# Aidenryan/GF_ORB_SLAM

Hardware: AMD Instinct MI355X
Metric: front-end fps (extract+match+GF-select) @ 752x480/1000 feats; pose-opt ms/iter (higher is better)
Workload: dtype u8/int32 (extract, match), f64 (GF, pose LM)

## Files before the change

### gf_orb_slam_amd/csrc/extract.hip

```cpp
#include <math.h>
#include <string.h>

#include <algorithm>
#include <cfloat>
#include <cmath>
#include <vector>

#include "common.h"
#include "libm_sincosf.h"
#include "orb_pattern.h"
#include "select.h"

#define GF_MAX_LEVELS 12

namespace {

__constant__ uint32_t c_pattern8[256];
__constant__ uint32_t c_ic_tab[256];

struct LevelGeom {
    int nlevels;
    int w[GF_MAX_LEVELS], h[GF_MAX_LEVELS];
    int pw[GF_MAX_LEVELS];
    long long off[GF_MAX_LEVELS];
// ... 601 lines not shown
            q[2] = row3(i2 * pitch + rsh[i2]);
        }
        int ie = rowi(ya + 2), se = rsh[ie];
        auto step = [&](int y, R3& u, R3& c, R3& d, R3& e) {
            e = row3(ie * pitch + se);
            const int in = rowi(y + 3);
            se = rsh[in];
            ie = in;
            const int mx = max(max(max(u.a, u.b), max(u.c, c.a)), max(max(c.c, d.a), max(d.b, d.c)));
            const bool keep = okc && c.b != 0 && c.b > mx;
            if (keep) atomicOr(&bits[(y * dw + x) >> 5], 1u << ((y * dw + x) & 31));
            cnt += __popcll(__ballot(keep));
        };
        for (int y = ya; y < yb; y += 4) {
            step(y, q[0], q[1], q[2], q[3]);
            if (y + 1 < yb) step(y + 1, q[1], q[2], q[3], q[0]);
            if (y + 2 < yb) step(y + 2, q[2], q[3], q[0], q[1]);
            if (y + 3 < yb) step(y + 3, q[3], q[0], q[1], q[2]);
        }
    }
    return cnt;
}

#ifndef FC_THREADS
#define FC_THREADS 256
#endif
constexpr int FC_NT = FC_THREADS, FC_NW = FC_THREADS / 64;
static_assert(FC_NT == 64 || FC_NT == 256 || FC_NT == 512, "k_fast_cells: 1, 4 or 8 waves");

template <int NW>
__device__ int block_scan_nw(int v, int* tmp, int& total) {
    const int lane = threadIdx.x & 63, wid = threadIdx.x >> 6;
    int wt;
    const int x = wave_scan_excl(v, wt);
    if (lane == 0) tmp[wid] = wt;
    __syncthreads();
    int base = 0;
    total = 0;
#pragma unroll
    for (int i = 0; i < NW; i++) {
        base += i < wid ? tmp[i] : 0;
        total += tmp[i];
    }
    __syncthreads();
    return base + x;
}
__device__ __forceinline__ void fc_sync() {
    if constexpr (FC_NT == 64) {
        __builtin_amdgcn_fence(__ATOMIC_RELEASE, "wavefront");
        __builtin_amdgcn_wave_barrier();
        __builtin_amdgcn_fence(__ATOMIC_ACQUIRE, "wavefront");
    } else {
        __syncthreads();
    }
}

struct FcLayout {
    int nq, ndw, pitch, wpr, nwords;
    size_t sc_bytes, bits_bytes, total;
};
__host__ __device__ inline FcLayout fc_layout(int dw, int dh, int w, int h) {
    FcLayout L;
    L.nq = (dw + 3) / 4;
    L.ndw = L.nq + 2;
    L.pitch = 4 * L.ndw;
    L.wpr = (dw + 31) / 32;
    L.nwords = dh * L.wpr;
    L.sc_bytes = (size_t)(dh + 2) * L.pitch;
    L.bits_bytes = 4 * (size_t)((L.nwords + 3) & ~3);
    L.total = L.sc_bytes + L.bits_bytes + (size_t)w * h;
    return L;
}

template <int NWV>
__device__ __forceinline__ int cell_nms4(const uint32_t* sc32, const FcLayout& Ly, uint32_t* bits, int dh, int th) {
    typedef unsigned short u2 __attribute__((ext_vector_type(2)));
    const int lane = threadIdx.x & 63, wv = threadIdx.x >> 6;
// ... 26 lines not shown
            const u2 vE = __builtin_elementwise_max(u.e, d.e), vO = __builtin_elementwise_max(u.o, d.o);
            const u2 vEL = __builtin_elementwise_max(u.el, d.el), vOR = __builtin_elementwise_max(u.orr, d.orr);
            const u2 mxE = __builtin_elementwise_max(__builtin_elementwise_max(vE, vEL),
                                                     __builtin_elementwise_max(vO, __builtin_elementwise_max(c.el, c.o)));
            const u2 mxO = __builtin_elementwise_max(__builtin_elementwise_max(vO, vOR),
                                                     __builtin_elementwise_max(vE, __builtin_elementwise_max(c.e, c.orr)));
            const u2 kE = __builtin_elementwise_min(__builtin_elementwise_sub_sat(c.e, mxE), ONE);
            const u2 kO = __builtin_elementwise_min(__builtin_elementwise_sub_sat(c.o, mxO), ONE);
            const uint32_t t = __builtin_bit_cast(uint32_t, kE) | (__builtin_bit_cast(uint32_t, kO) << 1);
            const uint32_t m = okq ? ((t & 3u) | ((t >> 14) & 12u)) : 0u;
            if (m) atomicOr(brow + (y - ya) * Ly.wpr, m << sh);
            cnt += __popc(m);
        };
        Q q0 = rowq(ya), q1 = rowq(ya + 1), q2;
        for (int y = ya; y < yb; y += 3) {
            step(y, q0, q1, q2);
            if (y + 1 < yb) step(y + 1, q1, q2, q0);
            if (y + 2 < yb) step(y + 2, q2, q0, q1);
        }
    }
    return gfd::warp_sum(cnt);
}

template <typename E>
__global__ __launch_bounds__(FC_NT) void k_fast_cells(Planes P, LevelGeom g, const uint8_t* __restrict__ score,
                                                    const CellInfo* __restrict__ cells, E* __restrict__ lists,
                                                    long long list_stride, int* __restrict__ counts, int fast_th,
                                                    int min_th) {
    gfd::ext_prio();
    extern __shared__ __align__(16) uint8_t smem[];
    __shared__ int s_cnt[2][FC_NW];
    __shared__ int scan_tmp[FC_NW];
    int cid, f;
    gfd::xcd_block(cid, f);
    const int tid = threadIdx.x;
    const CellInfo ci = cells[cid];
    if (ci.band) return;
    const int dw = ci.w - 6, dh = ci.h - 6;
    if (!ci.valid || dw <= 0 || dh <= 0) {
        if (tid == 0) counts[(long long)f * g.ncells + cid] = 0;
        return;
    }
    const FcLayout Ly = fc_layout(dw, dh, ci.w, ci.h);
    uint8_t* sc = smem;
    uint32_t* sc32 = reinterpret_cast<uint32_t*>(smem);
    uint32_t* bits = reinterpret_cast<uint32_t*>(smem + Ly.sc_bytes);
    const int l = ci.level, lw = g.pw[l];
    const uint8_t* SC = score + (long long)f * g.bslab + g.boff[l] + (long long)(ci.y0 + 3) * lw + ci.x0 + 3;
    {
        const uint32_t sh = (uint32_t)((uintptr_t)SC & 3u);
        const uint32_t* SCa = reinterpret_cast<const uint32_t*>((uintptr_t)SC & ~(uintptr_t)3);
        const int lw4 = lw >> 2, nrows = dh + 2;
        const int ndw = Ly.ndw, rstep = max(FC_NT / ndw, 1);
        const int j = tid % ndw, r0 = tid / ndw;
        const bool jdata = j >= 1 && j <= Ly.nq;
        uint32_t bmask = ~0u;
        if (jdata && dw - 4 * (j - 1) < 4) bmask = (1u << (8 * (dw - 4 * (j - 1)))) - 1u;
        constexpr int FC_LB = 8;
        for (int rb = r0; rb < nrows; rb += FC_LB * rstep) {
            uint32_t lo[FC_LB], hi[FC_LB];
            const int jc = min(max(j, 1), Ly.nq) - 1;
#pragma unroll
            for (int k = 0; k < FC_LB; k++) {
                const int rc = min(max(rb + k * rstep, 1), dh) - 1;
                const uint32_t* src = SCa + (long long)rc * lw4 + jc;
                lo[k] = gfd::ldg(src);
                hi[k] = gfd::ldg(src + 1);
            }
#pragma unroll
            for (int k = 0; k < FC_LB; k++) {
                const int r = rb + k * rstep;
                const bool data = jdata && r >= 1 && r <= dh;
                if (r < nrows && r0 < rstep)
                    sc32[r * ndw + j] = data ? __builtin_amdgcn_alignbyte(hi[k], lo[k], sh) & bmask : 0u;
            }
        }
    }
    for (int i = tid; i < Ly.nwords; i += FC_NT) bits[i] = 0;
    fc_sync();
    int c = cell_nms4<FC_NW>(sc32, Ly, bits, dh, fast_th);
    if ((tid & 63) == 0) s_cnt[0][tid >> 6] = c;
    fc_sync();
    int total = 0;
#pragma unroll
    for (int k = 0; k < FC_NW; k++) total += s_cnt[0][k];
    if (total <= 3) {
        uint8_t* roi = smem + Ly.sc_bytes + Ly.bits_bytes;
        int sstride;
        const uint8_t* Sl = level_plane(P, g, f, l, sstride) + (long long)ci.y0 * sstride + ci.x0;
        for (int i = tid; i < ci.w * ci.h; i += FC_NT) {
            const int r = pyr_div(i, 1.0f / (float)ci.w);
            roi[i] = gfd::ldg(Sl + (long long)r * sstride + (i - r * ci.w));
        }
        fc_sync();
        for (int i = tid; i < dw * dh; i += FC_NT) {
            const int y = pyr_div(i, 1.0f / (float)dw), x = i - y * dw;
            int cv[16];
            circle_vals(roi, ci.w, x + 3, y + 3, cv);
            const int M = fast_max_arc(roi[(y + 3) * ci.w + x + 3], cv);
            sc[(y + 1) * Ly.pitch + 4 + x] = M > min_th ? (uint8_t)M : 0;
        }
        for (int i = tid; i < Ly.nwords; i += FC_NT) bits[i] = 0;
        fc_sync();
        c = cell_nms4<FC_NW>(sc32, Ly, bits, dh, min_th);
        if ((tid & 63) == 0) s_cnt[1][tid >> 6] = c;
        fc_sync();
        total = 0;
#pragma unroll
        for (int k = 0; k < FC_NW; k++) total += s_cnt[1][k];
    }
    E* out = lists + (long long)f * list_stride + ci.cap_off;
    const int X0 = ci.x0 + 3, Y0 = ci.y0 + 3;
    int base = 0;
    for (int w0 = 0; w0 < Ly.nwords; w0 += FC_NT) {
        const int i = w0 + tid;
        uint32_t word = i < Ly.nwords ? bits[i] : 0u;
        int tot;
        int off;
        if constexpr (FC_NT == 64) {
            off = base + wave_scan_excl(__popc(word), tot);
        } else {
            off = base + block_scan_nw<FC_NW>(__popc(word), scan_tmp, tot);
        }
        if (word) {
            const int y = i / Ly.wpr, xw = 32 * (i - y * Ly.wpr);
            const uint8_t* srow = sc + (y + 1) * Ly.pitch + 4;
            while (word) {
                const int x = xw + __ffs(word) - 1;
                word &= word - 1;
                out[off++] = cell_entry<E>(srow[x] - 1, X0 + x, Y0 + y, P, g, f, l);
            }
        }
        base += tot;
    }
    if (tid == 0) counts[(long long)f * g.ncells + cid] = total;
}

template <typename E>
__global__ __launch_bounds__(256) void k_fast_cells_band(Planes P, LevelGeom g, const uint8_t* __restrict__ score,
                                                         const CellInfo* __restrict__ cells,
                                                         const int* __restrict__ band_ids, E* __restrict__ lists,
                                                         long long list_stride, int* __restrict__ counts, int fast_th,
                                                         int min_th) {
    gfd::ext_prio();
    extern __shared__ __align__(16) uint8_t smem[];
    __shared__ int s_cnt[4];
    __shared__ int scan_tmp[4];
    const int cid = band_ids[blockIdx.x], f = blockIdx.y, tid = threadIdx.x;
    const CellInfo ci = cells[cid];
    const int dw = ci.w - 6, dh = ci.h - 6, BH = ci.band;
    const int n = dw * dh, nwords = (n + 31) >> 5;
    const int ndw = (dw + 6) >> 2, pitch = 4 * ndw;
    uint32_t* bits = reinterpret_cast<uint32_t*>(smem);
    uint8_t* sc = smem + 16 * ((nwords + 3) / 4);
    uint8_t* rsh = sc + (BH + 3) * pitch;
    uint8_t* roi = rsh + ((BH + 3 + 15) & ~15);
    const int l = ci.level, lw = g.pw[l];
    const uint8_t* SC = score + (long long)f * g.bslab + g.boff[l] + (long long)(ci.y0 + 3) * lw + ci.x0 + 3;
// ... 74 lines not shown
#define SEL_MAX_CELLS 1024
#ifndef SEL_THREADS
#define SEL_THREADS 512
#endif
#define SEL_BUF 1024
#ifndef SEL_BUF_CELL
#define SEL_BUF_CELL 512
#endif
template <typename E>
struct SelWave {
    E* a;
    uint16_t *lp, *rp;
    int cap;
};
template <typename E>
constexpr size_t sel_wave_bytes(int cap) { return (size_t)cap * (sizeof(E) + 2 * sizeof(uint16_t)); }
template <typename E>
constexpr size_t sel_wave_lds() {
    return sel_wave_bytes<E>(SEL_BUF) + (SEL_THREADS / 64 - 1) * sel_wave_bytes<E>(SEL_BUF_CELL);
}
template <typename E>
constexpr size_t sel_lds(int maxnc) { return sel_wave_lds<E>() + sizeof(int) * (3 * (size_t)maxnc + 1) + (size_t)maxnc; }

__device__ __forceinline__ void wave_sync() {
    __builtin_amdgcn_fence(__ATOMIC_RELEASE, "wavefront");
    __builtin_amdgcn_wave_barrier();
    __builtin_amdgcn_fence(__ATOMIC_ACQUIRE, "wavefront");
}

template <typename E>
__device__ __forceinline__ int sel_resp(E e) { return Ent<E>::key(e); }

template <typename E>
__device__ __forceinline__ int wave_partition(const SelWave<E>& W, int lo, int hi, int P) {
    const int lane = threadIdx.x & 63;
    const unsigned long long lt = (1ull << lane) - 1ull;
    int nL = 0, nR = 0;
    for (int i0 = 0; i0 < hi - lo; i0 += 64) {
        const int i = lo + i0 + lane, j = hi - 1 - i0 - lane;
        const bool sl = i < hi && !(sel_resp(W.a[i]) > P);
        const bool sr = j >= lo && !(P > sel_resp(W.a[j]));
        const unsigned long long bl = __ballot(sl), br = __ballot(sr);
        if (sl) W.lp[nL + __popcll(bl & lt)] = (uint16_t)i;
        if (sr) W.rp[nR + __popcll(br & lt)] = (uint16_t)j;
        nL += __popcll(bl);
        nR += __popcll(br);
    }
    wave_sync();
    const int m = min(nL, nR);
    int ks = 0;
    for (int k0 = 0; k0 < m; k0 += 64) {
        const int k = k0 + lane;
// ... 411 lines not shown
        kp.angle = angle;
        kp.response = Ent<E>::response(e);
        kp.octave = l;
        kp.class_id = -1;
        kps[(long long)f * cap + k] = kp;
    }
}

}

struct gf_extractor {
    gf_ctx* ctx = nullptr;
    hipEvent_t stage_ev = nullptr;
    int stage_after = -1;
    int nfeatures = 0, nlevels = 0, fast_th = 20, min_th = 7, width = 0, height = 0, max_batch = 0;
    bool harris = false;
    float scale_factor = 1.2f;
    LevelGeom g{};
    std::vector<CellInfo> cells;
    std::vector<int> feat_per_level;
    int capacity = 0;
    long long list_stride = 0, lvl_stride = 0;
    size_t fast_lds = 0;
    size_t band_lds = 0;
    std::vector<int> band_cells;
    int* d_band = nullptr;
    int max_tiles = 0;
    uint8_t *d_pyr = nullptr, *d_blur = nullptr, *d_score = nullptr;
    uint32_t *d_xtab = nullptr, *d_ytab = nullptr;
    PyrGeom pg{};
    size_t pyr_lds = 0;
    int sel_maxnc = 0;
    int pyr_g = PYR_G;
    CellInfo* d_cells = nullptr;
    void *d_lists = nullptr, *d_lvl = nullptr;
    int *d_counts = nullptr, *d_lvl_counts = nullptr;
    uint8_t* d_img = nullptr;
    gf_keypoint* d_kps = nullptr;
    uint8_t* d_desc = nullptr;
    int* d_nout = nullptr;
    Planes last{};
};

static int cv_round_f(float v) { return (int)std::lrintf(v); }
static int cv_floor_f(float v) {
    int i = (int)v;
// ... 35 lines not shown
                 "level size out of supported range");
        if (l > 0) {
            g.off[l] = off;
            off += ((long long)g.pw[l] * g.h[l] + 255) & ~255LL;
        }
        g.boff[l] = boff;
        boff += ((long long)g.pw[l] * g.h[l] + 255) & ~255LL;
    }
    g.slab = off;
    g.bslab = boff;
    int t = 0;
    for (int l = 0; l < nl; l++) {
        g.tile_begin[l] = t;
        g.tiles_x[l] = (g.w[l] + BT_W - 1) / BT_W;
        t += g.tiles_x[l] * ((g.h[l] + BT_H - 1) / BT_H);
    }
    g.tile_begin[nl] = t;
    ex->max_tiles = t;

    ex->cells.clear();
    ex->sel_maxnc = 0;
    ex->band_cells.clear();
    ex->band_lds = 0;
    long long cap_off = 0, lvl_off = 0;
    size_t max_lds = 0;
    const float imageRatio = (float)g.w[0] / g.h[0];
    for (int l = 0; l < nl; l++) {
        const int nDesired = ex->feat_per_level[l];
        const int levelCols = (int)std::sqrt((float)nDesired / (5 * imageRatio));
        const int levelRows = (int)(imageRatio * levelCols);
        GF_CHECK(levelCols > 0 && levelRows > 0, GF_ERR_UNSUPPORTED, "level with an empty cell grid");
        const int minB = 16, maxBX = g.w[l] - 16, maxBY = g.h[l] - 16;
        const int W = maxBX - minB, H = maxBY - minB;
        const int cellW = (int)std::ceil((float)W / levelCols);
        const int cellH = (int)std::ceil((float)H / levelRows);
        const int nCells = levelRows * levelCols;
        GF_CHECK(nCells <= SEL_MAX_CELLS, GF_ERR_UNSUPPORTED, "too many cells per level");
        ex->sel_maxnc = std::max(ex->sel_maxnc, nCells);
        g.nfcell[l] = (int)std::ceil((float)nDesired / nCells);
        g.ndesired[l] = nDesired;
        g.cell_begin[l] = (int)ex->cells.size();
        g.lvl_off[l] = lvl_off;
        std::vector<int> iniXCol(levelCols, 0);
        float hY = cellH + 6;
        long long lvl_cap = 0;
        for (int i = 0; i < levelRows; i++) {
            const float iniY = minB + i * cellH - 3;
            bool rowSkip = false;
            if (i == levelRows - 1) {
                hY = maxBY + 3 - iniY;
                if (hY <= 0) rowSkip = true;
            }
            float hX = cellW + 6;
            for (int j = 0; j < levelCols; j++) {
                float iniX;
                if (i == 0) {
                    iniX = minB + j * cellW - 3;
                    iniXCol[j] = (int)iniX;
                } else
                    iniX = iniXCol[j];
                CellInfo ci{};
                ci.level = l;
                ci.valid = 0;
                if (!rowSkip) {
                    bool skip = false;
                    if (j == levelCols - 1) {
                        hX = maxBX + 3 - iniX;
                        if (hX <= 0) skip = true;
                    }
                    if (!skip) {
                        ci.x0 = (int)iniX;
                        ci.y0 = (int)iniY;
                        ci.w = (int)hX;
                        ci.h = (int)hY;
                        ci.valid = 1;
                        int dw = std::max(ci.w - 6, 0), dh = std::max(ci.h - 6, 0);
                        ci.cap = ((dw + 1) / 2) * ((dh + 1) / 2);
                        ci.cap_off = cap_off;
                        cap_off += ci.cap;
                        lvl_cap += ci.cap;
                        const size_t pitch = 4 * (size_t)((dw + 6) / 4), bits = 16 * (((size_t)dw * dh + 127) / 128);
                        const FcLayout fl = fc_layout(dw, dh, ci.w, ci.h);
                        const size_t lds = fl.total;
                        if (lds <= FC_LDS_MAX && fl.ndw <= FC_NT) {
                            max_lds = std::max(max_lds, lds);
                        } else {
                            auto band_lds = [&](size_t bh) {
                                return bits + (bh + 3) * pitch + ((bh + 3 + 15) & ~(size_t)15) + (bh + 8) * ci.w;
                            };
                            size_t bh = std::min<size_t>(dh, 64);
                            while (bh > 4 && band_lds(bh) > FC_BAND_LDS) bh /= 2;
                            GF_CHECK(band_lds(bh) <= FC_BAND_LDS, GF_ERR_UNSUPPORTED,
                                     "cell window too large even for the banded FAST kernel");
                            ci.band = (int)bh;
                            ex->band_cells.push_back((int)ex->cells.size());
                            ex->band_lds = std::max(ex->band_lds, band_lds(bh));
                        }
                        GF_CHECK(ci.x0 >= 0 && ci.y0 >= 0 && ci.x0 + ci.w <= g.w[l] && ci.y0 + ci.h <= g.h[l],
                                 GF_ERR_ARG, "cell ROI outside level");
                    }
                }
                ex->cells.push_back(ci);
            }
        }
        lvl_off += std::max(lvl_cap, (long long)nDesired);
    }
    g.cell_begin[nl] = (int)ex->cells.size();
    g.lvl_off[nl] = lvl_off;
    g.ncells = (int)ex->cells.size();
    ex->list_stride = cap_off;
    ex->lvl_stride = lvl_off;
    ex->fast_lds = max_lds;
    ex->capacity = 0;
    for (int l = 0; l < nl; l++) ex->capacity += ex->feat_per_level[l];
    return GF_OK;
}

static void resize_tables(int sw, int sh, int dw, int dh, std::vector<int2>& xt, std::vector<int2>& yt) {
    const int ONE = 2048;
    double scale_x = 1. / ((double)dw / sw), scale_y = 1. / ((double)dh / sh);
    xt.resize(dw);
    yt.resize(dh);
    for (int dx = 0; dx < dw; dx++) {
        float fx = (float)((dx + 0.5) * scale_x - 0.5);
        int sx = cv_floor_f(fx);
        fx -= sx;
        if (sx < 0) fx = 0, sx = 0;
        if (sx >= sw - 1) fx = 0, sx = sw - 1;
        int a0 = (short)cv_round_f((1.f - fx) * ONE), a1 = (short)cv_round_f(fx * ONE);
        xt[dx] = make_int2(sx, (a0 & 0xffff) | (a1 << 16));
    }
    for (int dy = 0; dy < dh; dy++) {
        float fy = (float)((dy + 0.5) * scale_y - 0.5);
        int sy = cv_floor_f(fy);
        fy -= sy;
        int b0 = (short)cv_round_f((1.f - fy) * ONE), b1 = (short)cv_round_f(fy * ONE);
        yt[dy] = make_int2(sy, (b0 & 0xffff) | (b1 << 16));
// ... 55 lines not shown
                    const PyrSpan& a = spx[(size_t)l * nbx + kx];
                    const PyrSpan& b = spy[(size_t)l * nby + ky];
                    const size_t pitch = (size_t)((a.hi - a.lo + 1 + 8 + 3) & ~3);
                    buf[l & 1] = std::max(buf[l & 1], pitch * (size_t)(b.hi - b.lo + 1));
                }
        buf[0] = (buf[0] + 15) & ~(size_t)15;
        if (mx <= 256 && buf[0] + buf[1] <= 64 * 1024) {
            pg.nbx = nbx;
            pg.nby = nby;
            pg.lds_a = (int)buf[0];
            lds = buf[0] + buf[1];
            return true;
        }
        if (mx > 256 || (double)g.w[0] / nbx >= (double)g.h[0] / nby) nbx++;
        else nby++;
    }
    return false;
}

static void free_extractor(gf_extractor* ex) {
    (void)hipFree(ex->d_pyr);
    (void)hipFree(ex->d_blur);
    (void)hipFree(ex->d_score);
    (void)hipFree(ex->d_xtab);
    (void)hipFree(ex->d_ytab);
    (void)hipFree(ex->d_cells);
    (void)hipFree(ex->d_band);
    (void)hipFree(ex->d_lists);
    (void)hipFree(ex->d_lvl);
    (void)hipFree(ex->d_counts);
    (void)hipFree(ex->d_lvl_counts);
    (void)hipFree(ex->d_img);
    (void)hipFree(ex->d_kps);
    (void)hipFree(ex->d_desc);
    (void)hipFree(ex->d_nout);
}

static int upload_constants(int device) {
    static unsigned long long done_mask = 0;
    if (done_mask & (1ull << device)) return GF_OK;
    {
        uint32_t p8[256];
        for (int i = 0; i < 256; i++) {
            uint32_t v = 0;
            for (int j = 0; j < 4; j++) {
                const int c = kOrbPattern31[4 * i + j];
// ... 45 lines not shown
    GF_CHECK(score_type == 0 || score_type == 1, GF_ERR_ARG, "scoreType: 0 HARRIS_SCORE, 1 FAST_SCORE");
    GF_CHECK(nlevels >= 1 && nlevels <= GF_MAX_LEVELS, GF_ERR_ARG, "nlevels out of range");
    GF_CHECK(nfeatures > 0 && scale_factor > 1.f && width > 0 && height > 0 && max_batch > 0, GF_ERR_ARG,
             "bad extractor parameters");
    GF_CHECK(fast_th >= 0 && fast_th < 255, GF_ERR_ARG, "bad FAST threshold");
    GF_HIP(hipSetDevice(ctx->device));
    int rc = upload_constants(ctx->device);
    if (rc) return rc;
    gf_extractor* ex = new gf_extractor();
    ex->ctx = ctx;
    ex->nfeatures = nfeatures;
    ex->scale_factor = scale_factor;
    ex->nlevels = nlevels;
    ex->fast_th = fast_th;
    ex->width = width;
    ex->height = height;
    ex->max_batch = max_batch;
    ex->harris = score_type == 0;
    rc = plan_extractor(ex);
    if (rc) {
        delete ex;
        return rc;
    }
    const LevelGeom& g = ex->g;
    auto cleanup = [&](hipError_t e) {
        free_extractor(ex);
        delete ex;
        return gf::fail(GF_ERR_HIP, std::string("extractor alloc: ") + hipGetErrorString(e));
    };
    hipError_t e;
#define ALLOC(p, bytes)                              \
    if ((e = hipMalloc((void**)&(p), (bytes))) != hipSuccess) return cleanup(e);
    ALLOC(ex->d_pyr, std::max<long long>(g.slab, 256) * max_batch);
    ALLOC(ex->d_blur, g.bslab * max_batch);
    ALLOC(ex->d_score, g.bslab * max_batch);
    ALLOC(ex->d_cells, sizeof(CellInfo) * ex->cells.size());
    const size_t esz = ex->harris ? sizeof(uint64_t) : sizeof(uint32_t);
    ALLOC(ex->d_lists, esz * ex->list_stride * max_batch);
    ALLOC(ex->d_lvl, esz * ex->lvl_stride * max_batch);
    ALLOC(ex->d_band, sizeof(int) * std::max<size_t>(ex->band_cells.size(), 1));
    ALLOC(ex->d_counts, sizeof(int) * g.ncells * max_batch);
    ALLOC(ex->d_lvl_counts, sizeof(int) * nlevels * max_batch);
    ALLOC(ex->d_img, (size_t)width * height);
    ALLOC(ex->d_kps, sizeof(gf_keypoint) * ex->capacity);
    ALLOC(ex->d_desc, 32 * (size_t)ex->capacity);
    ALLOC(ex->d_nout, sizeof(int));
    std::vector<std::vector<int2>> xts(nlevels), yts(nlevels);
    for (int l = 1; l < nlevels; l++) resize_tables(g.w[l - 1], g.h[l - 1], g.w[l], g.h[l], xts[l], yts[l]);
    std::vector<PyrSpan> spx, spy;
    if (nlevels > 1 && !pyr_plan(g, xts, yts, ex->pg, spx, spy, ex->pyr_lds)) {
        free_extractor(ex);
        delete ex;
        return gf::fail(GF_ERR_UNSUPPORTED, "scale factor too large for the pyramid blocks");
    }
    for (int l = 1; l < nlevels && ex->pyr_g > 1; l++)
        for (int k = 0; k < ex->pg.nbx; k++) {
            const PyrSpan& sp = spx[(size_t)l * ex->pg.nbx + k];
            for (int x0 = sp.lo; x0 <= sp.hi; x0 += PYR_G)
// ... 67 lines not shown
        }
        if (!ok) {
            free_extractor(ex);
            delete ex;
            return gf::fail(GF_ERR_UNSUPPORTED, "pyramid tables outside the k_pyramid record ranges");
        }
        ex->pg.rx = pack(rx, xrec);
        ex->pg.ry = pack(ry, yrec);
        ex->pg.lds_img = (int)((ex->pyr_lds + 15) & ~(size_t)15);
        ex->pyr_lds = ex->pg.lds_img + sizeof(uint32_t) * (size_t)(ex->pg.rx + ex->pg.ry);
    }
    ALLOC(ex->d_xtab, sizeof(uint32_t) * std::max<size_t>(xrec.size(), 1));
    ALLOC(ex->d_ytab, sizeof(uint32_t) * std::max<size_t>(yrec.size(), 1));
#undef ALLOC
    if (!xrec.empty()) {
        GF_HIP(hipMemcpy(ex->d_xtab, xrec.data(), sizeof(uint32_t) * xrec.size(), hipMemcpyHostToDevice));
        GF_HIP(hipMemcpy(ex->d_ytab, yrec.data(), sizeof(uint32_t) * yrec.size(), hipMemcpyHostToDevice));
        GF_HIP(hipFuncSetAttribute((const void*)k_pyramid<PYR_G>, hipFuncAttributeMaxDynamicSharedMemorySize,
                                   (int)ex->pyr_lds));
        GF_HIP(hipFuncSetAttribute((const void*)k_pyramid<1>, hipFuncAttributeMaxDynamicSharedMemorySize,
                                   (int)ex->pyr_lds));
    }
    GF_HIP(hipMemcpy(ex->d_cells, ex->cells.data(), sizeof(CellInfo) * ex->cells.size(), hipMemcpyHostToDevice));
    if (!ex->band_cells.empty())
        GF_HIP(hipMemcpy(ex->d_band, ex->band_cells.data(), sizeof(int) * ex->band_cells.size(),
                         hipMemcpyHostToDevice));
    if (ex->harris) {
        GF_HIP(hipFuncSetAttribute((const void*)k_select_cells<uint64_t>, hipFuncAttributeMaxDynamicSharedMemorySize,
                                   (int)(SEL_CW * sel_cell_wave_lds<uint64_t>(ex->sel_maxnc))));
        GF_HIP(hipFuncSetAttribute((const void*)k_fast_cells<uint64_t>, hipFuncAttributeMaxDynamicSharedMemorySize,
                                   (int)ex->fast_lds));
        GF_HIP(hipFuncSetAttribute((const void*)k_fast_cells_band<uint64_t>,
                                   hipFuncAttributeMaxDynamicSharedMemorySize, (int)ex->band_lds));
    } else {
        GF_HIP(hipFuncSetAttribute((const void*)k_select_cells<uint32_t>, hipFuncAttributeMaxDynamicSharedMemorySize,
                                   (int)(SEL_CW * sel_cell_wave_lds<uint32_t>(ex->sel_maxnc))));
        GF_HIP(hipFuncSetAttribute((const void*)k_fast_cells<uint32_t>, hipFuncAttributeMaxDynamicSharedMemorySize,
                                   (int)ex->fast_lds));
        GF_HIP(hipFuncSetAttribute((const void*)k_fast_cells_band<uint32_t>,
                                   hipFuncAttributeMaxDynamicSharedMemorySize, (int)ex->band_lds));
    }
    *out = ex;
    return GF_OK;
}

int gf_extractor_destroy(gf_extractor* ex) {
    if (!ex) return GF_OK;
    (void)hipSetDevice(ex->ctx->device);
    free_extractor(ex);
    delete ex;
    return GF_OK;
}

int gf_extractor_info(gf_extractor* ex, int* nlevels, float* scale_factor, int* features_per_level) {
    GF_CHECK(ex, GF_ERR_ARG, "null extractor");
    if (nlevels) *nlevels = ex->nlevels;
    if (scale_factor) *scale_factor = ex->scale_factor;
    if (features_per_level)
        for (int l = 0; l < ex->nlevels; l++) features_per_level[l] = ex->feat_per_level[l];
    return GF_OK;
// ... 44 lines not shown
                GF_LAUNCH(k_pyramid<1>, dim3(ex->pg.nbx * ex->pg.nby, nframes), PYR_NT, ex->pyr_lds, s, P, g, ex->pg,
                          ex->d_xtab, ex->d_ytab);
        }
    }
    if (ex->stage_ev && ex->stage_after == 0) GF_HIP(hipEventRecord(ex->stage_ev, s));
    {
        GF_PROF(ctx, s, "k_blur_fast");
        GF_LAUNCH(k_blur_fast, dim3(ex->max_tiles, nframes), 256, 0, s, P, g, ex->d_score, ex->fast_th);
    }
    if (ex->stage_ev && ex->stage_after == 1) GF_HIP(hipEventRecord(ex->stage_ev, s));
    return ex->harris ? select_describe<uint64_t>(ex, nframes, P, d_kps, d_desc, d_counts, cap, s)
                      : select_describe<uint32_t>(ex, nframes, P, d_kps, d_desc, d_counts, cap, s);
}

template <typename E>
static int select_describe(gf_extractor* ex, int nframes, Planes P, gf_keypoint* d_kps, uint8_t* d_desc,
                           int32_t* d_counts, int cap, hipStream_t s) {
    const LevelGeom& g = ex->g;
    gf_ctx* ctx = ex->ctx;
    E* lists = reinterpret_cast<E*>(ex->d_lists);
    E* lvl = reinterpret_cast<E*>(ex->d_lvl);
    {
        GF_PROF(ctx, s, "k_fast_cells");
        GF_LAUNCH(k_fast_cells<E>, dim3(g.ncells, nframes), FC_NT, ex->fast_lds, s, P, g, ex->d_score, ex->d_cells,
                  lists, ex->list_stride, ex->d_counts, ex->fast_th, ex->min_th);
        if (!ex->band_cells.empty())
            GF_LAUNCH(k_fast_cells_band<E>, dim3((int)ex->band_cells.size(), nframes), 256, ex->band_lds, s, P, g,
                      ex->d_score, ex->d_cells, ex->d_band, lists, ex->list_stride, ex->d_counts, ex->fast_th,
                      ex->min_th);
    }
    if (ex->stage_ev && ex->stage_after == 2) GF_HIP(hipEventRecord(ex->stage_ev, s));
    {
        GF_PROF(ctx, s, "k_select");
        GF_LAUNCH(k_select_cells<E>, dim3((g.ncells + SEL_CW - 1) / SEL_CW, nframes), 64 * SEL_CW,
                  SEL_CW * sel_cell_wave_lds<E>(ex->sel_maxnc), s, g, ex->d_cells, lists, ex->list_stride,
                  ex->d_counts, lvl, ex->lvl_stride, ex->d_lvl_counts, ex->sel_maxnc);
        GF_LAUNCH(k_select_level<E>, dim3(nframes, ex->nlevels), 64, sel_wave_bytes<E>(SEL_BUF), s, g, lvl,
                  ex->lvl_stride, ex->d_lvl_counts);
    }
    if (ex->stage_ev && ex->stage_after == 3) GF_HIP(hipEventRecord(ex->stage_ev, s));
    {
        GF_PROF(ctx, s, "k_describe");
        GF_LAUNCH(k_describe<E>, dim3((ex->capacity + 7) / 8, nframes), 256, 0, s, P, g, lvl, ex->lvl_stride,
                  ex->d_lvl_counts, d_kps, d_desc, d_counts, cap);
    }
    if (ex->stage_ev && ex->stage_after == 4) GF_HIP(hipEventRecord(ex->stage_ev, s));
    GF_HIP(hipGetLastError());
    return GF_OK;
// ... 79 lines not shown
```

Baseline: 127,100.

## Split FAST cell NMS into global tiled NMS, wave-per-cell listing, and retry kernel

Replaces the block-per-cell k_fast_cells kernel with three stages. A tiled k_nms_tiles kernel computes 3x3 NMS survivors over whole level rows into a global bitmask using DPP neighbour exchange and buffer loads. A wave-per-cell k_cell_lists kernel then compacts those survivors into per-cell lists. Cells with too few corners are queued to a separate k_cell_retry kernel that reruns FAST at the lower threshold. This removes per-cell LDS staging and block-wide syncs from the common path, at the cost of extra launches, a survivor bitmap in global memory, and host-side planning that requires non-overlapping cell windows.

After: 132,000, median of 6. 3.8% higher.

```diff
diff --git a/gf_orb_slam_amd/csrc/extract.hip b/gf_orb_slam_amd/csrc/extract.hip
--- a/gf_orb_slam_amd/csrc/extract.hip
+++ b/gf_orb_slam_amd/csrc/extract.hip
@@ -647,12 +647,6 @@
     return cnt;
 }
 
-#ifndef FC_THREADS
-#define FC_THREADS 256
-#endif
-constexpr int FC_NT = FC_THREADS, FC_NW = FC_THREADS / 64;
-static_assert(FC_NT == 64 || FC_NT == 256 || FC_NT == 512, "k_fast_cells: 1, 4 or 8 waves");
-
 template <int NW>
 __device__ int block_scan_nw(int v, int* tmp, int& total) {
     const int lane = threadIdx.x & 63, wid = threadIdx.x >> 6;
@@ -670,14 +664,10 @@
     __syncthreads();
     return base + x;
 }
-__device__ __forceinline__ void fc_sync() {
-    if constexpr (FC_NT == 64) {
-        __builtin_amdgcn_fence(__ATOMIC_RELEASE, "wavefront");
-        __builtin_amdgcn_wave_barrier();
-        __builtin_amdgcn_fence(__ATOMIC_ACQUIRE, "wavefront");
-    } else {
-        __syncthreads();
-    }
+__device__ __forceinline__ void wave_sync() {
+    __builtin_amdgcn_fence(__ATOMIC_RELEASE, "wavefront");
+    __builtin_amdgcn_wave_barrier();
+    __builtin_amdgcn_fence(__ATOMIC_ACQUIRE, "wavefront");
 }
 
 struct FcLayout {
@@ -750,118 +740,302 @@
     return gfd::warp_sum(cnt);
 }
 
+#define NMS_ROWS 32
+#define NMS_PF 4
+struct NmsTask {
+    int level, q0, y0, nrows;
+    uint32_t in, up, dn;
+    int xoff;
+};
+
+__global__ __launch_bounds__(256) void k_nms_tiles(LevelGeom g, const uint8_t* __restrict__ score,
+                                                   const NmsTask* __restrict__ tasks, int ntasks,
+                                                   const uint32_t* __restrict__ xtab, uint32_t* __restrict__ surv,
+                                                   int th, int* __restrict__ retry) {
+    gfd::ext_prio();
+    typedef unsigned short u2 __attribute__((ext_vector_type(2)));
+    if (blockIdx.x == 0 && blockIdx.y == 0 && threadIdx.x == 0) retry[0] = 0;
+    int blk, f;
+    gfd::xcd_block(blk, f);
+    const int lane = threadIdx.x & 63;
+    const int t = __builtin_amdgcn_readfirstlane(4 * blk + (int)(threadIdx.x >> 6));
+    if (t >= ntasks) return;
+    const NmsTask tk = tasks[t];
+    const int l = tk.level, pw = g.pw[l], nq = pw >> 2, h = g.h[l];
+    const int q = tk.q0 + lane;
+    const bool okq = q < nq;
+    const int qc = min(q, nq - 1);
+    const int qh = lane == 0 ? q - 1 : q + 1;
+    const int qhc = ((lane == 0 || lane == 63) && qh >= 0 && qh < nq) ? qh : qc;
+    const uint32_t xm = okq ? gfd::ldg(xtab + tk.xoff + qc) : 0u;
+    auto pair16 = [](uint32_t b, int i, int j) {
+        return ((b >> i) & 1u ? 0xffffu : 0u) | ((b >> j) & 1u ? 0xffff0000u : 0u);
+    };
+    const uint32_t mEL = pair16(xm, 4, 6), mOL = pair16(xm, 5, 7), mER = pair16(xm, 8, 10), mOR = pair16(xm, 9, 11);
+    const uint32_t inx = xm & 15u;
+    const unsigned short t1 = (unsigned short)max(th, 1);
+    const u2 T = {t1, t1}, ONE = {1, 1};
+    auto U = [](uint32_t v) { return __builtin_bit_cast(u2, v); };
+    auto V = [](u2 v) { return __builtin_bit_cast(uint32_t, v); };
+    const __amdgpu_buffer_rsrc_t rs = __builtin_amdgcn_make_buffer_rsrc(
+        const_cast<uint8_t*>(score + (long long)f * g.bslab + g.boff[l]), 0, pw * h, 0x00020000);
+    const int voff = 4 * qc, hoff = 4 * qhc;
+    struct Raw {
+        uint32_t b, hb;
+    };
+    auto load = [&](int y) -> Raw {
+        const int ro = min(max(y, 0), h - 1) * pw;
+        return Raw{(uint32_t)__builtin_amdgcn_raw_buffer_load_b32(rs, voff, ro, 0),
+                   (uint32_t)__builtin_amdgcn_raw_buffer_load_b32(rs, hoff, ro, 0)};
+    };
+    struct Row {
+        u2 e, o, hE, hO, vE, vO;
+    };
+    auto make = [&](Raw r) -> Row {
+        const uint32_t b = r.b;
+        const uint32_t a = (uint32_t)__builtin_amdgcn_update_dpp((int)r.hb, (int)b, 0x138, 0xf, 0xf, false);
+        const uint32_t c = (uint32_t)__builtin_amdgcn_update_dpp((int)r.hb, (int)b, 0x130, 0xf, 0xf, false);
+        Row x;
+        x.e = __builtin_elementwise_sub_sat(U(__builtin_amdgcn_perm(0u, b, 0x0c020c00u)), T);
+        x.o = __builtin_elementwise_sub_sat(U(__builtin_amdgcn_perm(0u, b, 0x0c030c01u)), T);
+        const u2 el = __builtin_elementwise_sub_sat(U(__builtin_amdgcn_perm(a, b, 0x0c010c07u)), T);
+        const u2 orr = __builtin_elementwise_sub_sat(U(__builtin_amdgcn_perm(c, b, 0x0c040c02u)), T);
+        x.hE = __builtin_elementwise_max(U(V(el) & mEL), U(V(x.o) & mER));
+        x.hO = __builtin_elementwise_max(U(V(x.e) & mOL), U(V(orr) & mOR));
+        x.vE = __builtin_elementwise_max(x.hE, x.e);
+        x.vO = __builtin_elementwise_max(x.hO, x.o);
+        return x;
+    };
+    const int spw = pw >> 5;
+    uint32_t* srow = surv + (long long)f * (g.bslab >> 5) + (g.boff[l] >> 5) + (long long)tk.y0 * spw + (q >> 3);
+    const bool st = okq && (lane & 7) == 7;
+    const int sh = 4 * (lane & 7);
+    auto put = [&](int r, u2 mxE, u2 mxO, const Row& c) {
+        const uint32_t k = V(__builtin_elementwise_min(__builtin_elementwise_sub_sat(c.e, mxE), ONE)) |
+                           (V(__builtin_elementwise_min(__builtin_elementwise_sub_sat(c.o, mxO), ONE)) << 1);
+        uint32_t v = ((k | (k >> 14)) & inx) << sh;
+        v |= (uint32_t)__builtin_amdgcn_update_dpp(0, (int)v, 0x111, 0xf, 0xf, true);
+        v |= (uint32_t)__builtin_amdgcn_update_dpp(0, (int)v, 0x112, 0xf, 0xf, true);
+        v |= (uint32_t)__builtin_amdgcn_update_dpp(0, (int)v, 0x114, 0xf, 0xf, true);
+        if (st) srow[(long long)r * spw] = v;
+    };
+    auto step = [&](int r, const Row& u, const Row& c, const Row& d) {
+        const bool up = (tk.up >> r) & 1u, dn = (tk.dn >> r) & 1u;
+        if (up && dn) {
+            put(r, __builtin_elementwise_max(c.hE, __builtin_elementwise_max(u.vE, d.vE)),
+                __builtin_elementwise_max(c.hO, __builtin_elementwise_max(u.vO, d.vO)), c);
+        } else if ((tk.in >> r) & 1u) {
+            const uint32_t su = up ? ~0u : 0u, sd = dn ? ~0u : 0u;
+            put(r, __builtin_elementwise_max(c.hE, __builtin_elementwise_max(U(V(u.vE) & su), U(V(d.vE) & sd))),
+                __builtin_elementwise_max(c.hO, __builtin_elementwise_max(U(V(u.vO) & su), U(V(d.vO) & sd))), c);
+        } else if (st) {
+            srow[(long long)r * spw] = 0u;
+        }
+    };
+    Row u = make(load(tk.y0 - 1)), c = make(load(tk.y0));
+    Raw cur[NMS_PF], nxt[NMS_PF];
+#pragma unroll
+    for (int k = 0; k < NMS_PF; k++) cur[k] = load(tk.y0 + 1 + k);
+    for (int r0 = 0; r0 < tk.nrows; r0 += NMS_PF) {
+#pragma unroll
+        for (int k = 0; k < NMS_PF; k++) nxt[k] = load(tk.y0 + 1 + r0 + NMS_PF + k);
+#pragma unroll
+        for (int k = 0; k < NMS_PF; k++) {
+            if (r0 + k < tk.nrows) {
+                const Row d = make(cur[k]);
+                step(r0 + k, u, c, d);
+                u = c;
+                c = d;
+            }
+            cur[k] = nxt[k];
+        }
+    }
+}
+
+#define CL_NW 5
+#define CL_NS 2
+struct CellWin {
+    int dw, dh, l, lw, spw, X0, Y0, wpr, nwords;
+    float rwpr;
+    const uint32_t* SV;
+    const uint8_t* SC;
+};
+__device__ __forceinline__ CellWin cell_win(const CellInfo& ci, const LevelGeom& g, const uint8_t* score,
+                                            const uint32_t* surv, int f) {
+    CellWin c;
+    c.dw = ci.w - 6;
+    c.dh = ci.h - 6;
+    c.l = ci.level;
+    c.lw = g.pw[c.l];
+    c.spw = c.lw >> 5;
+    c.X0 = ci.x0 + 3;
+    c.Y0 = ci.y0 + 3;
+    c.wpr = (c.dw + 31) >> 5;
+    c.nwords = c.dh * c.wpr;
+    c.rwpr = 1.0f / (float)c.wpr;
+    c.SV = surv + (long long)f * (g.bslab >> 5) + (g.boff[c.l] >> 5) + (long long)c.Y0 * c.spw;
+    c.SC = score + (long long)f * g.bslab + g.boff[c.l] + (long long)c.Y0 * c.lw + c.X0;
+    return c;
+}
+__device__ __forceinline__ uint32_t cell_word(const CellWin& c, int i) {
+    const int ic = min(i, c.nwords - 1);
+    const int y = pyr_div(ic, c.rwpr), k = ic - y * c.wpr;
+    const int xs = c.X0 + 32 * k, wi = xs >> 5, n = c.dw - 32 * k;
+    const uint32_t* p = c.SV + (long long)y * c.spw;
+    const uint32_t lo = gfd::ldg(p + wi), hi = gfd::ldg(p + min(wi + 1, c.spw - 1));
+    const uint32_t w = __builtin_amdgcn_alignbit(hi, lo, (uint32_t)(xs & 31));
+    return i < c.nwords ? (n >= 32 ? w : w & ((1u << n) - 1u)) : 0u;
+}
+
 template <typename E>
-__global__ __launch_bounds__(FC_NT) void k_fast_cells(Planes P, LevelGeom g, const uint8_t* __restrict__ score,
+__global__ __launch_bounds__(256) void k_cell_lists(Planes P, LevelGeom g, const uint8_t* __restrict__ score,
+                                                    const uint32_t* __restrict__ surv,
                                                     const CellInfo* __restrict__ cells, E* __restrict__ lists,
-                                                    long long list_stride, int* __restrict__ counts, int fast_th,
+                                                    long long list_stride, int* __restrict__ counts,
+                                                    int* __restrict__ retry) {
+    gfd::ext_prio();
+    int blk, f;
+    gfd::xcd_block(blk, f);
+    const int lane = threadIdx.x & 63;
+    const int cid = __builtin_amdgcn_readfirstlane(4 * blk + (int)(threadIdx.x >> 6));
+    if (cid >= g.ncells) return;
+    const CellInfo ci = cells[cid];
+    if (ci.band) return;
+    if (!ci.valid || ci.w - 6 <= 0 || ci.h - 6 <= 0) {
+        if (lane == 0) counts[(long long)f * g.ncells + cid] = 0;
+        return;
+    }
+    const CellWin c = cell_win(ci, g, score, surv, f);
+    uint32_t w[CL_NW];
+#pragma unroll
+    for (int j = 0; j < CL_NW; j++) w[j] = cell_word(c, 64 * j + lane);
+    int off[CL_NW], tot[CL_NW], total = 0;
+#pragma unroll
+    for (int j = 0; j < CL_NW; j++) {
+        off[j] = wave_scan_excl(__popc(w[j]), tot[j]);
+        total += tot[j];
+    }
+    int rest = 0;
+    for (int i0 = 64 * CL_NW; i0 < c.nwords; i0 += 64) rest += __popc(cell_word(c, i0 + lane));
+    if (c.nwords > 64 * CL_NW) total += gfd::warp_sum(rest);
+    if (total <= 3) {
+        if (lane == 0) retry[1 + atomicAdd(retry, 1)] = f * g.ncells + cid;
+        return;
+    }
+    E* out = lists + (long long)f * list_stride + ci.cap_off;
+    int sx[CL_NW][CL_NS], sy[CL_NW], sS[CL_NW][CL_NS];
+#pragma unroll
+    for (int j = 0; j < CL_NW; j++) {
+        const int i = 64 * j + lane;
+        const int y = pyr_div(i, c.rwpr), xw = 32 * (i - y * c.wpr);
+        sy[j] = y;
+        uint32_t word = w[j];
+#pragma unroll
+        for (int s = 0; s < CL_NS; s++) {
+            const bool has = word != 0u;
+            const int x = xw + __ffs(word) - 1;
+            word &= word - 1;
+            sx[j][s] = has ? x : -1;
+            sS[j][s] = gfd::ldg(c.SC + (has ? (long long)y * c.lw + x : 0ll));
+        }
+        w[j] = word;
+    }
+    int base = 0;
+#pragma unroll
+    for (int j = 0; j < CL_NW; j++) {
+        int o = base + off[j];
+#pragma unroll
+        for (int s = 0; s < CL_NS; s++)
+            if (sx[j][s] >= 0) out[o++] = cell_entry<E>(sS[j][s] - 1, c.X0 + sx[j][s], c.Y0 + sy[j], P, g, f, c.l);
+        uint32_t word = w[j];
+        while (word) {
+            const int x = 32 * (64 * j + lane - sy[j] * c.wpr) + __ffs(word) - 1;
+            word &= word - 1;
+            const int S = gfd::ldg(c.SC + (long long)sy[j] * c.lw + x) - 1;
+            out[o++] = cell_entry<E>(S, c.X0 + x, c.Y0 + sy[j], P, g, f, c.l);
+        }
+        base += tot[j];
+    }
+    for (int i0 = 64 * CL_NW; i0 < c.nwords; i0 += 64) {
+        const int i = i0 + lane;
+        uint32_t word = cell_word(c, i);
+        int t;
+        int o = base + wave_scan_excl(__popc(word), t);
+        const int y = pyr_div(i, c.rwpr), xw = 32 * (i - y * c.wpr);
+        while (word) {
+            const int x = xw + __ffs(word) - 1;
+            word &= word - 1;
+            const int S = gfd::ldg(c.SC + (long long)y * c.lw + x) - 1;
+            out[o++] = cell_entry<E>(S, c.X0 + x, c.Y0 + y, P, g, f, c.l);
+        }
+        base += t;
+    }
+    if (lane == 0) counts[(long long)f * g.ncells + cid] = total;
+}
+
+template <typename E>
+__global__ __launch_bounds__(256) void k_cell_retry(Planes P, LevelGeom g, const CellInfo* __restrict__ cells,
+                                                    E* __restrict__ lists, long long list_stride,
+                                                    int* __restrict__ counts, const int* __restrict__ retry,
                                                     int min_th) {
     gfd::ext_prio();
     extern __shared__ __align__(16) uint8_t smem[];
-    __shared__ int s_cnt[2][FC_NW];
-    __shared__ int scan_tmp[FC_NW];
-    int cid, f;
-    gfd::xcd_block(cid, f);
+    __shared__ int s_cnt[4];
+    __shared__ int scan_tmp[4];
     const int tid = threadIdx.x;
-    const CellInfo ci = cells[cid];
-    if (ci.band) return;
-    const int dw = ci.w - 6, dh = ci.h - 6;
-    if (!ci.valid || dw <= 0 || dh <= 0) {
-        if (tid == 0) counts[(long long)f * g.ncells + cid] = 0;
-        return;
-    }
-    const FcLayout Ly = fc_layout(dw, dh, ci.w, ci.h);
-    uint8_t* sc = smem;
-    uint32_t* sc32 = reinterpret_cast<uint32_t*>(smem);
-    uint32_t* bits = reinterpret_cast<uint32_t*>(smem + Ly.sc_bytes);
-    const int l = ci.level, lw = g.pw[l];
-    const uint8_t* SC = score + (long long)f * g.bslab + g.boff[l] + (long long)(ci.y0 + 3) * lw + ci.x0 + 3;
-    {
-        const uint32_t sh = (uint32_t)((uintptr_t)SC & 3u);
-        const uint32_t* SCa = reinterpret_cast<const uint32_t*>((uintptr_t)SC & ~(uintptr_t)3);
-        const int lw4 = lw >> 2, nrows = dh + 2;
-        const int ndw = Ly.ndw, rstep = max(FC_NT / ndw, 1);
-        const int j = tid % ndw, r0 = tid / ndw;
-        const bool jdata = j >= 1 && j <= Ly.nq;
-        uint32_t bmask = ~0u;
-        if (jdata && dw - 4 * (j - 1) < 4) bmask = (1u << (8 * (dw - 4 * (j - 1)))) - 1u;
-        constexpr int FC_LB = 8;
-        for (int rb = r0; rb < nrows; rb += FC_LB * rstep) {
-            uint32_t lo[FC_LB], hi[FC_LB];
-            const int jc = min(max(j, 1), Ly.nq) - 1;
-#pragma unroll
-            for (int k = 0; k < FC_LB; k++) {
-                const int rc = min(max(rb + k * rstep, 1), dh) - 1;
-                const uint32_t* src = SCa + (long long)rc * lw4 + jc;
-                lo[k] = gfd::ldg(src);
-                hi[k] = gfd::ldg(src + 1);
-            }
-#pragma unroll
-            for (int k = 0; k < FC_LB; k++) {
-                const int r = rb + k * rstep;
-                const bool data = jdata && r >= 1 && r <= dh;
-                if (r < nrows && r0 < rstep)
-                    sc32[r * ndw + j] = data ? __builtin_amdgcn_alignbyte(hi[k], lo[k], sh) & bmask : 0u;
-            }
-        }
-    }
-    for (int i = tid; i < Ly.nwords; i += FC_NT) bits[i] = 0;
-    fc_sync();
-    int c = cell_nms4<FC_NW>(sc32, Ly, bits, dh, fast_th);
-    if ((tid & 63) == 0) s_cnt[0][tid >> 6] = c;
-    fc_sync();
-    int total = 0;
-#pragma unroll
-    for (int k = 0; k < FC_NW; k++) total += s_cnt[0][k];
-    if (total <= 3) {
+    const int nq = retry[0];
+    for (int it = blockIdx.x; it < nq; it += gridDim.x) {
+        const int id = retry[1 + it], f = id / g.ncells, cid = id - f * g.ncells;
+        const CellInfo ci = cells[cid];
+        const int dw = ci.w - 6, dh = ci.h - 6, l = ci.level;
+        const FcLayout Ly = fc_layout(dw, dh, ci.w, ci.h);
+        uint8_t* sc = smem;
+        uint32_t* sc32 = reinterpret_cast<uint32_t*>(smem);
+        uint32_t* bits = reinterpret_cast<uint32_t*>(smem + Ly.sc_bytes);
         uint8_t* roi = smem + Ly.sc_bytes + Ly.bits_bytes;
+        __syncthreads();
+        for (int i = tid; i < (dh + 2) * Ly.ndw; i += 256) sc32[i] = 0u;
+        for (int i = tid; i < Ly.nwords; i += 256) bits[i] = 0u;
         int sstride;
         const uint8_t* Sl = level_plane(P, g, f, l, sstride) + (long long)ci.y0 * sstride + ci.x0;
-        for (int i = tid; i < ci.w * ci.h; i += FC_NT) {
+        for (int i = tid; i < ci.w * ci.h; i += 256) {
             const int r = pyr_div(i, 1.0f / (float)ci.w);
             roi[i] = gfd::ldg(Sl + (long long)r * sstride + (i - r * ci.w));
         }
-        fc_sync();
-        for (int i = tid; i < dw * dh; i += FC_NT) {
+        __syncthreads();
+        for (int i = tid; i < dw * dh; i += 256) {
             const int y = pyr_div(i, 1.0f / (float)dw), x = i - y * dw;
             int cv[16];
             circle_vals(roi, ci.w, x + 3, y + 3, cv);
             const int M = fast_max_arc(roi[(y + 3) * ci.w + x + 3], cv);
             sc[(y + 1) * Ly.pitch + 4 + x] = M > min_th ? (uint8_t)M : 0;
         }
-        for (int i = tid; i < Ly.nwords; i += FC_NT) bits[i] = 0;
-        fc_sync();
-        c = cell_nms4<FC_NW>(sc32, Ly, bits, dh, min_th);
-        if ((tid & 63) == 0) s_cnt[1][tid >> 6] = c;
-        fc_sync();
-        total = 0;
-#pragma unroll
-        for (int k = 0; k < FC_NW; k++) total += s_cnt[1][k];
-    }
-    E* out = lists + (long long)f * list_stride + ci.cap_off;
-    const int X0 = ci.x0 + 3, Y0 = ci.y0 + 3;
-    int base = 0;
-    for (int w0 = 0; w0 < Ly.nwords; w0 += FC_NT) {
-        const int i = w0 + tid;
-        uint32_t word = i < Ly.nwords ? bits[i] : 0u;
-        int tot;
-        int off;
-        if constexpr (FC_NT == 64) {
-            off = base + wave_scan_excl(__popc(word), tot);
-        } else {
-            off = base + block_scan_nw<FC_NW>(__popc(word), scan_tmp, tot);
-        }
-        if (word) {
-            const int y = i / Ly.wpr, xw = 32 * (i - y * Ly.wpr);
-            const uint8_t* srow = sc + (y + 1) * Ly.pitch + 4;
-            while (word) {
-                const int x = xw + __ffs(word) - 1;
-                word &= word - 1;
-                out[off++] = cell_entry<E>(srow[x] - 1, X0 + x, Y0 + y, P, g, f, l);
-            }
-        }
-        base += tot;
-    }
-    if (tid == 0) counts[(long long)f * g.ncells + cid] = total;
+        __syncthreads();
+        const int cw = cell_nms4<4>(sc32, Ly, bits, dh, min_th);
+        if ((tid & 63) == 0) s_cnt[tid >> 6] = cw;
+        __syncthreads();
+        const int total = s_cnt[0] + s_cnt[1] + s_cnt[2] + s_cnt[3];
+        E* out = lists + (long long)f * list_stride + ci.cap_off;
+        const int X0 = ci.x0 + 3, Y0 = ci.y0 + 3;
+        int base = 0;
+        for (int w0 = 0; w0 < Ly.nwords; w0 += 256) {
+            const int i = w0 + tid;
+            uint32_t word = i < Ly.nwords ? bits[i] : 0u;
+            int tot;
+            int off = base + block_scan_nw<4>(__popc(word), scan_tmp, tot);
+            if (word) {
+                const int y = i / Ly.wpr, xw = 32 * (i - y * Ly.wpr);
+                const uint8_t* srow = sc + (y + 1) * Ly.pitch + 4;
+                while (word) {
+                    const int x = xw + __ffs(word) - 1;
+                    word &= word - 1;
+                    out[off++] = cell_entry<E>(srow[x] - 1, X0 + x, Y0 + y, P, g, f, l);
+                }
+            }
+            base += tot;
+        }
+        if (tid == 0) counts[(long long)f * g.ncells + cid] = total;
+    }
 }
 
 template <typename E>
@@ -982,12 +1156,6 @@
 template <typename E>
 constexpr size_t sel_lds(int maxnc) { return sel_wave_lds<E>() + sizeof(int) * (3 * (size_t)maxnc + 1) + (size_t)maxnc; }
 
-__device__ __forceinline__ void wave_sync() {
-    __builtin_amdgcn_fence(__ATOMIC_RELEASE, "wavefront");
-    __builtin_amdgcn_wave_barrier();
-    __builtin_amdgcn_fence(__ATOMIC_ACQUIRE, "wavefront");
-}
-
 template <typename E>
 __device__ __forceinline__ int sel_resp(E e) { return Ent<E>::key(e); }
 
@@ -1445,6 +1613,11 @@
     int capacity = 0;
     long long list_stride = 0, lvl_stride = 0;
     size_t fast_lds = 0;
+    int* d_retry = nullptr;
+    std::vector<int> level_cols;
+    std::vector<NmsTask> nms_tasks;
+    NmsTask* d_nms_tasks = nullptr;
+    uint32_t *d_nms_xtab = nullptr, *d_surv = nullptr;
     size_t band_lds = 0;
     std::vector<int> band_cells;
     int* d_band = nullptr;
@@ -1526,6 +1699,7 @@
     ex->sel_maxnc = 0;
     ex->band_cells.clear();
     ex->band_lds = 0;
+    ex->level_cols.clear();
     long long cap_off = 0, lvl_off = 0;
     size_t max_lds = 0;
     const float imageRatio = (float)g.w[0] / g.h[0];
@@ -1545,6 +1719,7 @@
         g.ndesired[l] = nDesired;
         g.cell_begin[l] = (int)ex->cells.size();
         g.lvl_off[l] = lvl_off;
+        ex->level_cols.push_back(levelCols);
         std::vector<int> iniXCol(levelCols, 0);
         float hY = cellH + 6;
         long long lvl_cap = 0;
@@ -1586,7 +1761,7 @@
                         const size_t pitch = 4 * (size_t)((dw + 6) / 4), bits = 16 * (((size_t)dw * dh + 127) / 128);
                         const FcLayout fl = fc_layout(dw, dh, ci.w, ci.h);
                         const size_t lds = fl.total;
-                        if (lds <= FC_LDS_MAX && fl.ndw <= FC_NT) {
+                        if (lds <= FC_LDS_MAX && fl.ndw <= 256) {
                             max_lds = std::max(max_lds, lds);
                         } else {
                             auto band_lds = [&](size_t bh) {
@@ -1617,6 +1792,76 @@
     ex->fast_lds = max_lds;
     ex->capacity = 0;
     for (int l = 0; l < nl; l++) ex->capacity += ex->feat_per_level[l];
+    return GF_OK;
+}
+
+static int nms_plan(gf_extractor* ex, std::vector<uint32_t>& xtab) {
+    const LevelGeom& g = ex->g;
+    ex->nms_tasks.clear();
+    xtab.clear();
+    for (int l = 0; l < g.nlevels; l++) {
+        const int w = g.w[l], h = g.h[l], pw = g.pw[l], cols = ex->level_cols[l];
+        std::vector<int> colid(pw + 1, -1), rowid(h + 1, -1);
+        for (int k = g.cell_begin[l]; k < g.cell_begin[l + 1]; k++) {
+            const CellInfo& ci = ex->cells[k];
+            const int i = (k - g.cell_begin[l]) / cols, j = (k - g.cell_begin[l]) % cols;
+            if (!ci.valid || ci.w - 6 <= 0 || ci.h - 6 <= 0) continue;
+            for (int x = ci.x0 + 3; x < ci.x0 + ci.w - 3; x++) {
+                GF_CHECK(x >= 0 && x < w && (colid[x] == -1 || colid[x] == j), GF_ERR_UNSUPPORTED,
+                         "cell windows overlap in x");
+                colid[x] = j;
+            }
+            for (int y = ci.y0 + 3; y < ci.y0 + ci.h - 3; y++) {
+                GF_CHECK(y >= 0 && y < h && (rowid[y] == -1 || rowid[y] == i), GF_ERR_UNSUPPORTED,
+                         "cell windows overlap in y");
+                rowid[y] = i;
+            }
+        }
+        for (int k = g.cell_begin[l]; k < g.cell_begin[l + 1]; k++) {
+            const CellInfo& ci = ex->cells[k];
+            const int i = (k - g.cell_begin[l]) / cols, j = (k - g.cell_begin[l]) % cols;
+            if (!ci.valid || ci.w - 6 <= 0 || ci.h - 6 <= 0) continue;
+            GF_CHECK(std::count(colid.begin(), colid.end(), j) == ci.w - 6 &&
+                         std::count(rowid.begin(), rowid.end(), i) == ci.h - 6,
+                     GF_ERR_UNSUPPORTED, "cell windows are not a product of column and row ranges");
+        }
+        const int xoff = (int)xtab.size(), nq = pw / 4;
+        for (int q = 0; q < nq; q++) {
+            uint32_t e = 0;
+            for (int b = 0; b < 4; b++) {
+                const int c = 4 * q + b;
+                if (colid[c] < 0) continue;
+                e |= 1u << b;
+                if (c >= 1 && colid[c - 1] == colid[c]) e |= 1u << (4 + b);
+                if (colid[c + 1] == colid[c]) e |= 1u << (8 + b);
+            }
+            xtab.push_back(e);
+        }
+        int ylo = 0, yhi = h;
+        while (ylo < h && rowid[ylo] < 0) ylo++;
+        while (yhi > ylo && rowid[yhi - 1] < 0) yhi--;
+        for (int q0 = 0; q0 < nq; q0 += 64) {
+            bool any = false;
+            for (int q = q0; q < std::min(q0 + 64, nq); q++) any = any || (xtab[xoff + q] & 15u);
+            if (!any) continue;
+            for (int y0 = ylo; y0 < yhi; y0 += NMS_ROWS) {
+                NmsTask t{};
+                t.level = l;
+                t.q0 = q0;
+                t.y0 = y0;
+                t.nrows = std::min(NMS_ROWS, yhi - y0);
+                t.xoff = xoff;
+                for (int r = 0; r < t.nrows; r++) {
+                    const int y = y0 + r;
+                    if (rowid[y] < 0) continue;
+                    t.in |= 1u << r;
+                    if (y >= 1 && rowid[y - 1] == rowid[y]) t.up |= 1u << r;
+                    if (rowid[y + 1] == rowid[y]) t.dn |= 1u << r;
+                }
+                ex->nms_tasks.push_back(t);
+            }
+        }
+    }
     return GF_OK;
 }
 
@@ -1718,6 +1963,10 @@
     (void)hipFree(ex->d_pyr);
     (void)hipFree(ex->d_blur);
     (void)hipFree(ex->d_score);
+    (void)hipFree(ex->d_surv);
+    (void)hipFree(ex->d_retry);
+    (void)hipFree(ex->d_nms_tasks);
+    (void)hipFree(ex->d_nms_xtab);
     (void)hipFree(ex->d_xtab);
     (void)hipFree(ex->d_ytab);
     (void)hipFree(ex->d_cells);
@@ -1809,6 +2058,12 @@
         delete ex;
         return rc;
     }
+    std::vector<uint32_t> nms_xtab;
+    rc = nms_plan(ex, nms_xtab);
+    if (rc) {
+        delete ex;
+        return rc;
+    }
     const LevelGeom& g = ex->g;
     auto cleanup = [&](hipError_t e) {
         free_extractor(ex);
@@ -1821,6 +2076,10 @@
     ALLOC(ex->d_pyr, std::max<long long>(g.slab, 256) * max_batch);
     ALLOC(ex->d_blur, g.bslab * max_batch);
     ALLOC(ex->d_score, g.bslab * max_batch);
+    ALLOC(ex->d_surv, g.bslab / 8 * max_batch);
+    ALLOC(ex->d_retry, sizeof(int) * ((size_t)g.ncells * max_batch + 1));
+    ALLOC(ex->d_nms_tasks, sizeof(NmsTask) * std::max<size_t>(ex->nms_tasks.size(), 1));
+    ALLOC(ex->d_nms_xtab, sizeof(uint32_t) * std::max<size_t>(nms_xtab.size(), 1));
     ALLOC(ex->d_cells, sizeof(CellInfo) * ex->cells.size());
     const size_t esz = ex->harris ? sizeof(uint64_t) : sizeof(uint32_t);
     ALLOC(ex->d_lists, esz * ex->list_stride * max_batch);
@@ -1934,20 +2193,27 @@
                                    (int)ex->pyr_lds));
     }
     GF_HIP(hipMemcpy(ex->d_cells, ex->cells.data(), sizeof(CellInfo) * ex->cells.size(), hipMemcpyHostToDevice));
+    GF_HIP(hipMemset(ex->d_surv, 0, (size_t)(g.bslab / 8) * max_batch));
+    GF_HIP(hipMemset(ex->d_retry, 0, sizeof(int)));
+    if (!ex->nms_tasks.empty()) {
+        GF_HIP(hipMemcpy(ex->d_nms_tasks, ex->nms_tasks.data(), sizeof(NmsTask) * ex->nms_tasks.size(),
+                         hipMemcpyHostToDevice));
+        GF_HIP(hipMemcpy(ex->d_nms_xtab, nms_xtab.data(), sizeof(uint32_t) * nms_xtab.size(), hipMemcpyHostToDevice));
+    }
     if (!ex->band_cells.empty())
         GF_HIP(hipMemcpy(ex->d_band, ex->band_cells.data(), sizeof(int) * ex->band_cells.size(),
                          hipMemcpyHostToDevice));
     if (ex->harris) {
         GF_HIP(hipFuncSetAttribute((const void*)k_select_cells<uint64_t>, hipFuncAttributeMaxDynamicSharedMemorySize,
                                    (int)(SEL_CW * sel_cell_wave_lds<uint64_t>(ex->sel_maxnc))));
-        GF_HIP(hipFuncSetAttribute((const void*)k_fast_cells<uint64_t>, hipFuncAttributeMaxDynamicSharedMemorySize,
+        GF_HIP(hipFuncSetAttribute((const void*)k_cell_retry<uint64_t>, hipFuncAttributeMaxDynamicSharedMemorySize,
                                    (int)ex->fast_lds));
         GF_HIP(hipFuncSetAttribute((const void*)k_fast_cells_band<uint64_t>,
                                    hipFuncAttributeMaxDynamicSharedMemorySize, (int)ex->band_lds));
     } else {
         GF_HIP(hipFuncSetAttribute((const void*)k_select_cells<uint32_t>, hipFuncAttributeMaxDynamicSharedMemorySize,
                                    (int)(SEL_CW * sel_cell_wave_lds<uint32_t>(ex->sel_maxnc))));
-        GF_HIP(hipFuncSetAttribute((const void*)k_fast_cells<uint32_t>, hipFuncAttributeMaxDynamicSharedMemorySize,
+        GF_HIP(hipFuncSetAttribute((const void*)k_cell_retry<uint32_t>, hipFuncAttributeMaxDynamicSharedMemorySize,
                                    (int)ex->fast_lds));
         GF_HIP(hipFuncSetAttribute((const void*)k_fast_cells_band<uint32_t>,
                                    hipFuncAttributeMaxDynamicSharedMemorySize, (int)ex->band_lds));
@@ -2038,8 +2304,16 @@
     E* lvl = reinterpret_cast<E*>(ex->d_lvl);
     {
         GF_PROF(ctx, s, "k_fast_cells");
-        GF_LAUNCH(k_fast_cells<E>, dim3(g.ncells, nframes), FC_NT, ex->fast_lds, s, P, g, ex->d_score, ex->d_cells,
-                  lists, ex->list_stride, ex->d_counts, ex->fast_th, ex->min_th);
+        if (!ex->nms_tasks.empty())
+            GF_LAUNCH(k_nms_tiles, dim3(((int)ex->nms_tasks.size() + 3) / 4, nframes), 256, 0, s, g, ex->d_score,
+                      ex->d_nms_tasks, (int)ex->nms_tasks.size(), ex->d_nms_xtab, ex->d_surv, ex->fast_th,
+                      ex->d_retry);
+        GF_LAUNCH(k_cell_lists<E>, dim3((g.ncells + 3) / 4, nframes), 256, 0, s, P, g, ex->d_score, ex->d_surv,
+                  ex->d_cells, lists, ex->list_stride, ex->d_counts, ex->d_retry);
+        if (ex->fast_lds)
+            GF_LAUNCH(k_cell_retry<E>, dim3((unsigned)std::min<long long>((long long)g.ncells * nframes, 2048)), 256,
+                      ex->fast_lds, s, P, g, ex->d_cells, lists, ex->list_stride, ex->d_counts, ex->d_retry,
+                      ex->min_th);
         if (!ex->band_cells.empty())
             GF_LAUNCH(k_fast_cells_band<E>, dim3((int)ex->band_cells.size(), nframes), 256, ex->band_lds, s, P, g,
                       ex->d_score, ex->d_cells, ex->d_band, lists, ex->list_stride, ex->d_counts, ex->fast_th,
```
